# mayataka/robotoc

Hardware: AMD Instinct MI355X
Metric: riccati_sweeps_per_sec (higher is better)
Workload: dtype f64; 1 GPU; anymal_trot_N40 (nv=18,nu=12, 47 grids: 2 lifts + 2 impacts, switching constraints ns=6), 4096 DISTINCT OCP instances per GPU (randomised stage data and dx0), backward+forward Riccati sweep; per_gpu_batch=4096, stages=47, parallelism=instances sharded, dp1

## Files before the change

robotoc_amd/csrc/kernel_set.hpp:

```cpp
#pragma once
#include <cstring>

#include "../../include/rtoc.h"
#include "condense.hpp"
#include "state_equation.hpp"
#include "unconstr_dynamics.hpp"
#include "friction_cone.hpp"
#include "kkt_error.hpp"
#include "integrate_solution.hpp"
#include "riccati_backward.hpp"
#include "riccati_backward_rs.hpp"
#include "riccati_backward_rv.hpp"
#include "riccati_backward_rw.hpp"
#include "riccati_backward_rw2.hpp"
#include "condense_rv.hpp"
#include "riccati_scan.hpp"
#include "riccati_forward.hpp"
#include "unconstr_riccati.hpp"

namespace rtoc {

typedef void (*bwd_fn)(BwdArgs);
typedef void (*fwd_fn)(FwdArgs);
typedef void (*fill_fn)(FillArgs);
typedef void (*ud_fn)(UdArgs);
typedef void (*cone_fn)(ConeArgs);
typedef void (*cond_fn)(CondArgs);
typedef void (*expd_fn)(ExpArgs);
typedef void (*scan_fn)(ScanArgs);
typedef void (*fscan_fn)(FwdScanArgs);
typedef void (*stoscan_fn)(StoScanArgs);
typedef void (*ur_fn)(UrArgs);
constexpr size_t kernel_abi_stamp() {
  size_t h = 1469598103934665603ull;
  const size_t parts[] = {sizeof(BwdArgs), sizeof(FwdArgs), sizeof(FillArgs), sizeof(UdArgs), sizeof(ConeArgs), sizeof(CondArgs),
                          sizeof(ExpArgs), sizeof(ScanArgs), sizeof(FwdScanArgs), sizeof(UrArgs), sizeof(StoScanArgs)};
  for (size_t v : parts) h = (h ^ v) * 1099511628211ull;
  return h;
}

struct KernelSet {
  int nv, nu, ns;
  int nvariants;
  bwd_fn bwd[4];
  int bwd_waves[4];
  int bwd_lds[4];
  int bwd_inst[4];
  bwd_fn bwd_sa;
  bwd_fn bwd_rv;
  bwd_fn bwd_rv_sa;
  bwd_fn bwd_rv_sto;
  int bwd_rv_lds;
  bwd_fn bwd_rw;
  int bwd_rw_lds;
  int bwd_rw_threads;
  rtoc_record_layout kl, rl, dl, cl;
  fwd_fn fwd;
  int fwd_threads;
  fill_fn fill;
  ud_fn ucond, uexp;
  ur_fn ubwd, ufwd;
  cone_fn ccond, cexp;
  cone_fn wcond, wexp;
  cond_fn cond;
  cond_fn cond_split, mjt;
  int mjt_lds;
  int cond_threads, cond_lds, cond_split_lds;
  int cond_fuses_cones;
  int cond_fused_default;
  cond_fn cond_rv_nc;
  cond_fn cond_rv;
  int cond_rv_lds;
  int cond_rv_cones;
  expd_fn expd;
  int expd_threads, expd_lds;
  scan_fn scan_elt, scan_comb;
  int scan_elt_lds, scan_comb_lds, scan_comb_threads;
  int scan_elt_stride, scan_ps_stride, scan_ps_soff;
  int scan_policy_variant;
  fscan_fn fscan_elt, fscan_comb, fscan_fin;
  int fscan_lds;
  stoscan_fn sto_prep, sto_vec;
  int sto_prep_lds, sto_vec_lds, sto_vec_threads, sto_scr_stride;
};

template <int NV, int NU, int NS, int NW0, int NW1>
inline KernelSet make_set() {
  KernelSet k;
  memset(&k, 0, sizeof(k));
  k.nv = NV;
  k.nu = NU;
  k.ns = NS;
  k.nvariants = 2;
  for (int v = 0; v < 4; ++v) k.bwd_inst[v] = 1;
  k.kl = StaticLayout<NV, NU, NS>::make().kkt;
  k.rl = StaticLayout<NV, NU, NS>::make().ric;
  k.bwd[0] = riccati_backward_kernel<NV, NU, NS, NW0>;
  k.bwd_waves[0] = NW0;
  k.bwd_lds[0] = BwdCfg<NV, NU, NS, NW0>::LDS_BYTES;
  k.bwd[1] = riccati_backward_kernel<NV, NU, NS, NW1>;
  k.bwd_waves[1] = NW1;
  k.bwd_lds[1] = BwdCfg<NV, NU, NS, NW1>::LDS_BYTES;
  if constexpr (2 * NV + 1 <= 64 && NU + 3 <= 16) {
    k.bwd[2] = riccati_backward_rs_kernel<NV, NU, NS>;
    k.bwd_waves[2] = 2;
    k.bwd_lds[2] = BwdCfg<NV, NU, NS, 2>::LDS_BYTES;
    k.nvariants = 3;
    if (4 * BwdCfg<NV, NU, NS, 2>::LDS_BYTES + 64 <= 160 * 1024) {
      k.bwd[3] = riccati_backward_rs4_kernel<NV, NU, NS>;
      k.bwd_waves[3] = 8;
      k.bwd_lds[3] = 4 * BwdCfg<NV, NU, NS, 2>::LDS_BYTES + 64;
      k.bwd_inst[3] = 4;
      k.nvariants = 4;
      if constexpr (NV % 4 == 2 && NV > NU) k.bwd_sa = riccati_backward_rs4_kernel<NV, NU, NS, true>;
    }
  }
  if constexpr (RvCfg<NV, NU>::OK) {
    k.bwd_rv = riccati_backward_rv_kernel<NV, NU, NS, false>;
    if constexpr (NV % 16 == 2 && RvCfg<NV, NU>::T == 3 && NV - NU > 0 && NV - NU <= 8 && (NV - NU) % 2 == 0)
    {
      k.bwd_rv_sa = riccati_backward_rv_kernel<NV, NU, NS, true>;
      k.bwd_rv_sto = riccati_backward_rv_kernel<NV, NU, NS, true, true>;
    }
    k.bwd_rv_lds = rv_lds_bytes<NV, NU, NS>();
  }
  if constexpr (RwCfg<NV, NU>::OK) {
    k.bwd_rw = riccati_backward_rw_kernel<NV, NU, NS>;
    k.bwd_rw_lds = RwLds<NV, NU, NS>::BYTES;
    k.bwd_rw_threads = 64;
  } else if constexpr (RwCfg<NV, NU>::OK2) {
    k.bwd_rw = riccati_backward_rw2_kernel<NV, NU, NS>;
    k.bwd_rw_lds = Rw2Lds<NV, NU, NS>::BYTES;
    k.bwd_rw_threads = 128;
  }
  constexpr int NWF = (2 * NV + NU + 63) / 64;
  if constexpr (NWF == 1)
    k.fwd = riccati_forward_kernel<NV, NU, NS, 1>;
  else
    k.fwd = riccati_forward_mw_kernel<NV, NU, NS, NWF>;
  k.fwd_threads = 64 * NWF;
  k.dl = StaticLayout<NV, NU, NS>::make().dir;
  k.cl = StaticLayout<NV, NU, NS>::make().cdd;
  k.fill = unconstr_fill_kernel<NV>;
  k.ucond = unconstr_condense_kernel<NV>;
  k.uexp = unconstr_expand_kernel<NV>;
  if constexpr (NU == NV && NS == 0 && 2 * NV + 1 <= 64) {
    if constexpr (NV <= 8) k.ubwd = unconstr_riccati_backward_kernel<NV>;
    else k.ubwd = unconstr_riccati_backward_lds_kernel<NV>;
    k.ufwd = unconstr_riccati_forward_kernel<NV>;
  }
  k.ccond = cone_condense_kernel<NV, NS>;
  k.cexp = cone_expand_kernel<NV, NS>;
  k.wcond = wrench_condense_kernel<NV, NS>;
  k.wexp = wrench_expand_kernel<NV, NS>;
  constexpr int NF = NS;
  k.cond = condense_kernel<NV, NU, NF, NS>;
  k.cond_split = condense_kernel<NV, NU, NF, NS, true>;
  k.mjt = mjtjinv_kernel<NV, NU, NF, NS>;
  k.mjt_lds = MjCfg<NV, NF>::LDS_BYTES;
  k.cond_threads = CondCfg<NV, NU, NF, NS>::NT;
  k.cond_lds = CondCfg<NV, NU, NF, NS>::LDS_BYTES;
  k.cond_split_lds = CondCfg<NV, NU, NF, NS, true>::LDS_BYTES;
  k.cond_fuses_cones = CondCfg<NV, NU, NF, NS>::FUSE ? 1 : 0;
  k.cond_fused_default = (CondCfg<NV, NU, NF, NS>::FUSE && CondCfg<NV, NU, NF, NS>::ITEMS >= 5) ? 1 : 0;
  k.cond_rv = nullptr;
  k.cond_rv_nc = nullptr;
  k.cond_rv_lds = 0;
  k.cond_rv_cones = 0;
  if constexpr (CrvCfg<NV, NU, NF, NS>::OK) {
    k.cond_rv = condense_rv_kernel<NV, NU, NF, NS>;
    k.cond_rv_nc = condense_rv_kernel<NV, NU, NF, NS, false>;
    k.cond_rv_lds = CrvCfg<NV, NU, NF, NS>::LDS_BYTES;
    k.cond_rv_cones = CrvCfg<NV, NU, NF, NS>::CONES ? 1 : 0;
  }
  static_assert(!(NV == 18 && NU == 12 && NS == 12) ||
                    (CondCfg<NV, NU, NF, NS, true>::ITEMS >= 5 && CondCfg<NV, NU, NF, NS, true>::MIN_WAVES == 4 && MjCfg<NV, NF>::ITEMS >= 10),
                "LDS carve of the split condensation grew past its granule budget");
  k.expd = expand_kernel<NV, NU, NF, NS>;
  k.expd_threads = 64;
  k.expd_lds = ExpCfg<NV, NU, NF>::LDS_BYTES;
  k.scan_elt = scan_element_kernel<NV, NU, NS>;
  k.scan_comb = scan_combine_kernel<NV>;
  k.scan_elt_lds = scan::ElementCfg<NV, NU, NS>::LDS_BYTES;
  k.scan_comb_threads = scan_comb_nt(NV);
  k.scan_comb_lds = scan::CombineCfg<NV, scan_comb_nt(NV)>::LDS_BYTES;
  k.scan_elt_stride = scan::EltLayout<NV>::STRIDE;
  k.scan_ps_stride = scan::EltLayout<NV>::PS_STRIDE;
  k.scan_ps_soff = scan::EltLayout<NV>::PS_S;
  k.scan_policy_variant = 1;
  k.fscan_elt = fwd_scan_element_kernel<NV, NU, NS>;
  k.fscan_comb = fwd_scan_combine_kernel<NV, NU, NS>;
  k.fscan_fin = fwd_scan_finish_kernel<NV, NU, NS>;
  k.fscan_lds = scan::FwdCfg<NV, NU>::LDS_BYTES;
  k.sto_prep = scan_sto_prep_kernel<NV, NU, NS>;
  k.sto_vec = scan_sto_vector_kernel<NV, NU, NS>;
  k.sto_prep_lds = scan::StoPrepCfg<NV, NU, NS>::LDS_DOUBLES * (int)sizeof(double);
  k.sto_vec_lds = scan::StoVecCfg<NV, NU, NS>::LDS_BYTES;
  k.sto_vec_threads = scan_sto_vec_nt(NV);
  k.sto_scr_stride = scan::StoScratch<NV, NU, NS>::STRIDE;
  static_assert(scan::StoVecCfg<NV, NU, NS>::LDS_BYTES <= 160 * 1024, "the vector pass keeps one grid point's bundle in LDS");
  static_assert(scan::CombineCfg<NV, scan_comb_nt(NV)>::LDS_BYTES <= 160 * 1024, "combination scratch must fit the LDS of a CU");
  return k;
}


}
```

robotoc_amd/csrc/riccati_forward.hpp:

```cpp
#pragma once
#include "device_utils.hpp"
#include "../../include/rtoc.h"

namespace rtoc {

#ifndef FWD_UNROLL
#define FWD_UNROLL 18
#endif
#ifndef FWD_REST_PARTS
#define FWD_REST_PARTS 2
#endif
#ifndef FWD_HEAD
#define FWD_HEAD 8
#endif

struct FwdArgs {
  const double* kkt;
  const double* ric;
  double* dir;
  const double* dx0;
  const rtoc_grid* grid;
  int nstages;
  int batch;
  int first;
};

template <int NWF>
__device__ __forceinline__ void fwd_sync() {
  if constexpr (NWF == 1)
    asm volatile("s_waitcnt lgkmcnt(0)" ::: "memory");
  else
    asm volatile("s_waitcnt lgkmcnt(0)\n\ts_barrier" ::: "memory");
}

template <int NV, int NU, int NS, int NWF>
__global__ __launch_bounds__(64 * NWF, 4) void riccati_forward_kernel(FwdArgs a) {
  constexpr int NX = 2 * NV, NT = 64 * NWF;
  constexpr bool MFOLD = NS > 0 && NX + NU + NS <= NT;
  static_assert(NX + NU <= NT, "one thread per row of [Fxx;K]");
  __shared__ double sDx[2][NX + 8];
  __shared__ double sDu[NU + 8];
  __shared__ double sRed[8];
  extern __shared__ int sGridTab[];
  const int tid = threadIdx.x;
  const int b = a.first + blockIdx.x;
  if (b >= a.batch) return;
  for (int st = tid; st < a.nstages; st += NT) {
    const rtoc_grid* gp = a.grid + st;
    sGridTab[st] = (gp->type & 15) | ((gp->sto != 0) << 4) | ((gp->sto_next != 0) << 5) |
                   ((gp->switching_constraint != 0) << 6) | (gp->dims << 8);
  }
  const int N = a.nstages - 1;
  constexpr rtoc_layout SL = StaticLayout<NV, NU, NS>::make();
  constexpr rtoc_record_layout KL = SL.kkt, RL = SL.ric, DL = SL.dir;
  const double* kb = a.kkt + (size_t)b * a.nstages * KL.stride;
  const double* rb = a.ric + (size_t)b * a.nstages * RL.stride;
  double* db = a.dir + (size_t)b * a.nstages * DL.stride;

  if (tid < NX) {
    const double v = a.dx0 ? a.dx0[(size_t)b * NX + tid] : db[DL.off[RTOC_DIR_DX] + tid];
    sDx[0][tid] = v;
    if (a.dx0) db[DL.off[RTOC_DIR_DX] + tid] = v;
  }
  __syncthreads();
  double dts = 0.0, dtsn = 0.0;
  {
    const rtoc_grid g0 = a.grid[0];
    if (g0.sto) {
      if (tid == 0) {
        double acc = 0.0;
        for (int k = 0; k < NX; ++k) acc += rb[RL.off[RTOC_RIC_DTSDX] + k] * sDx[0][k];
        sRed[0] = acc + rb[RL.off[RTOC_RIC_SCAL] + RTOC_RIC_SCAL_DTS0];
      }
      __syncthreads();
      dtsn = sRed[0];
      __syncthreads();
    }
  }
  int cur = 0;
  struct GridBits { int type, sto, sto_next, switching_constraint, dims; };
  struct StageRows {
    const double *pa, *pp, *pv, *ps;
    int sa;
  };
  auto stage_rows = [&](int st) {
    const int gb = __builtin_amdgcn_readfirstlane(sGridTab[st]);
    const bool imp = (gb & 15) == RTOC_GRID_IMPACT;
    const bool xrow = tid < NX;
    const bool krow = !imp && tid >= NX && tid < NX + NU;
    const bool mrow = MFOLD && ((gb >> 6) & 1) && tid >= NX + NU && tid < NX + NU + (gb >> 8);
    const int u = krow ? tid - NX : 0;
    const int m = mrow ? tid - NX - NU : 0;
    const int t = xrow ? tid : 0;
    const double* kr = kb + (size_t)st * KL.stride;
    const double* rr = rb + (size_t)st * RL.stride;
    StageRows r;
    r.pa = xrow ? kr + KL.off[RTOC_KKT_FXX] + tid
                : (mrow ? rr + RL.off[RTOC_RIC_M] + m : rr + RL.off[RTOC_RIC_K] + (size_t)u * NX);
    r.sa = xrow ? NX : (mrow ? NS : 1);
    r.pp = rr + RL.off[RTOC_RIC_P] + t;
    r.pv = xrow ? kr + KL.off[RTOC_KKT_FX] + tid : (mrow ? rr + RL.off[RTOC_RIC_MV] + m : rr + RL.off[RTOC_RIC_KV] + u);
    r.ps = rr + RL.off[RTOC_RIC_S] + t;
    return r;
  };
  constexpr int H = NX < FWD_HEAD ? NX : FWD_HEAD;
  double ha[H], hp[H], vec, sv;
  {
    const StageRows r0 = stage_rows(0);
#pragma unroll
    for (int j = 0; j < H; ++j) {
      ha[j] = r0.pa[j * r0.sa];
      hp[j] = r0.pp[j * NX];
    }
    vec = *r0.pv;
    sv = *r0.ps;
  }
  for (int st = 0; st < N; ++st) {
    const int gb = __builtin_amdgcn_readfirstlane(sGridTab[st]);
    const GridBits g = {gb & 15, (gb >> 4) & 1, (gb >> 5) & 1, (gb >> 6) & 1, gb >> 8};
    const bool impact = g.type == RTOC_GRID_IMPACT, lift = g.type == RTOC_GRID_LIFT;
    const bool sto = g.sto != 0, sto_next = g.sto_next != 0;
    const double* kr = kb + (size_t)st * KL.stride;
    const double* rr = rb + (size_t)st * RL.stride;
    double* dr = db + (size_t)st * DL.stride;
    const double* dx = sDx[cur];
    double* dxn = sDx[cur ^ 1];

    if (impact || lift) {
      dts = dtsn;
      dtsn = 0.0;
      if (lift && sto_next) {
        if (tid == 0) {
          double acc = 0.0;
          for (int k = 0; k < NX; ++k) acc += rr[RL.off[RTOC_RIC_DTSDX] + k] * dx[k];
          acc += rr[RL.off[RTOC_RIC_SCAL] + RTOC_RIC_SCAL_DTS0];
          if (sto) acc += rr[RL.off[RTOC_RIC_SCAL] + RTOC_RIC_SCAL_DTSDTS] * dts;
          sRed[0] = acc;
        }
        fwd_sync<NWF>();
        dtsn = sRed[0];
        fwd_sync<NWF>();
      }
    }

    const bool xrow = tid < NX;
    const bool krow = !impact && tid >= NX && tid < NX + NU;
    const bool mrow = MFOLD && g.switching_constraint && tid >= NX + NU && tid < NX + NU + g.dims;
    const int u = krow ? tid - NX : 0;
    const int m = mrow ? tid - NX - NU : 0;
    const StageRows r = stage_rows(st);
    double bv[NU];
    double acc_a = 0.0, acc_p = 0.0;
#pragma unroll
    for (int j = 0; j < H; ++j) {
      const double x = dx[j];
      acc_a += ha[j] * x;
      acc_p += hp[j] * x;
    }
#pragma unroll((NX - H + FWD_REST_PARTS - 1) / FWD_REST_PARTS > 0 ? (NX - H + FWD_REST_PARTS - 1) / FWD_REST_PARTS : 1)
    for (int j = H; j < NX; ++j) {
      const double x = dx[j];
      acc_a += r.pa[j * r.sa] * x;
      acc_p += r.pp[j * NX] * x;
    }
    {
      const double* Bv = kr + KL.off[RTOC_KKT_FVU] + ((tid >= NV && tid < NX) ? tid - NV : 0);
#pragma unroll
      for (int c = 0; c < NU; ++c) bv[c] = Bv[c * NV];
    }
    double vec_n, sv_n;
    {
      const StageRows rn = stage_rows(st + 1);
#pragma unroll
      for (int j = 0; j < H; ++j) {
        ha[j] = rn.pa[j * rn.sa];
        hp[j] = rn.pp[j * NX];
      }
      vec_n = *rn.pv;
      sv_n = *rn.ps;
    }
    if (krow) {
      double du = acc_a + vec;
      if (sto) {
        du += rr[RL.off[RTOC_RIC_T] + u] * (dtsn - dts);
        if (sto_next) du -= rr[RL.off[RTOC_RIC_W] + u] * dtsn;
      }
      sDu[u] = du;
      dr[DL.off[RTOC_DIR_DU] + u] = du;
    }
    fwd_sync<NWF>();
    if (xrow) {
      double v = vec + acc_a;
      if (!impact) {
        if (tid >= NV) {
#pragma unroll
          for (int c = 0; c < NU; ++c) v += bv[c] * sDu[c];
        }
        if (sto) v += kr[KL.off[RTOC_KKT_FFX] + tid] * (dtsn - dts);
      }
      dxn[tid] = v;
      (dr + DL.stride)[DL.off[RTOC_DIR_DX] + tid] = v;
    }
    if (impact && sto_next) {
      fwd_sync<NWF>();
      if (tid == 0) {
        double acc = 0.0;
        for (int k = 0; k < NX; ++k) acc += rr[RL.off[RTOC_RIC_DTSDX] + k] * dxn[k];
        acc += rr[RL.off[RTOC_RIC_SCAL] + RTOC_RIC_SCAL_DTS0];
        if (sto) acc += rr[RL.off[RTOC_RIC_SCAL] + RTOC_RIC_SCAL_DTSDTS] * dts;
        sRed[0] = acc;
      }
      fwd_sync<NWF>();
      dtsn = sRed[0];
    }
    if (tid < NX) {
      double lam = acc_p - sv;
      if (sto) {
        if (impact) {
          lam -= rr[RL.off[RTOC_RIC_PHI] + tid] * dtsn;
        } else {
          lam += rr[RL.off[RTOC_RIC_PSI] + tid] * (dtsn - dts);
          if (sto_next) lam -= rr[RL.off[RTOC_RIC_PHI] + tid] * dtsn;
        }
      }
      dr[DL.off[RTOC_DIR_DLMDGMM] + tid] = lam;
    }
    if constexpr (MFOLD) {
      if (mrow) {
        double acc = acc_a + vec;
        if (sto) {
          acc += rr[RL.off[RTOC_RIC_MT] + m] * (dtsn - dts);
          if (sto_next) acc -= rr[RL.off[RTOC_RIC_MTN] + m] * dtsn;
        }
        dr[DL.off[RTOC_DIR_DXI] + m] = acc;
      }
    } else if (NS > 0 && g.switching_constraint && tid < g.dims) {
      const double* M = rr + RL.off[RTOC_RIC_M] + tid;
      double acc = 0.0;
      for (int j = 0; j < NX; ++j) acc += M[j * NS] * dx[j];
      acc += rr[RL.off[RTOC_RIC_MV] + tid];
      if (sto) {
        acc += rr[RL.off[RTOC_RIC_MT] + tid] * (dtsn - dts);
        if (sto_next) acc -= rr[RL.off[RTOC_RIC_MTN] + tid] * dtsn;
      }
      dr[DL.off[RTOC_DIR_DXI] + tid] = acc;
    }
    if (tid == 0) {
      dr[DL.off[RTOC_DIR_DTS] + 0] = dts;
      dr[DL.off[RTOC_DIR_DTS] + 1] = dtsn;
    }
    fwd_sync<NWF>();
    cur ^= 1;
    vec = vec_n;
    sv = sv_n;
  }
  {
    const double* rr = rb + (size_t)N * RL.stride;
    double* dr = db + (size_t)N * DL.stride;
    const double* dx = sDx[cur];
    if (tid < NX) {
      const double* P = rr + RL.off[RTOC_RIC_P] + tid;
      double acc = 0.0;
#pragma unroll FWD_UNROLL
      for (int j = 0; j < NX; ++j) acc += P[j * NX] * dx[j];
      dr[DL.off[RTOC_DIR_DLMDGMM] + tid] = acc - rr[RL.off[RTOC_RIC_S] + tid];
    }
    if (tid == 0) {
      dr[DL.off[RTOC_DIR_DTS] + 0] = dts;
      dr[DL.off[RTOC_DIR_DTS] + 1] = dtsn;
    }
  }
}

template <int NV, int NU, int NS, int NWF>
__global__ __launch_bounds__(64 * NWF) void riccati_forward_mw_kernel(FwdArgs a) {
  constexpr int NX = 2 * NV, NT = 64 * NWF;
  static_assert(NX + NU <= NT, "one thread per row of [Fxx;K]");
  __shared__ double sDx[2][NX + 8];
  __shared__ double sDu[NU + 8];
  __shared__ double sRed[8];
  const int tid = threadIdx.x;
  const int b = a.first + blockIdx.x;
  if (b >= a.batch) return;
  const int N = a.nstages - 1;
  constexpr rtoc_layout SL = StaticLayout<NV, NU, NS>::make();
  constexpr rtoc_record_layout KL = SL.kkt, RL = SL.ric, DL = SL.dir;
  const double* kb = a.kkt + (size_t)b * a.nstages * KL.stride;
  const double* rb = a.ric + (size_t)b * a.nstages * RL.stride;
  double* db = a.dir + (size_t)b * a.nstages * DL.stride;

  if (tid < NX) {
    const double v = a.dx0 ? a.dx0[(size_t)b * NX + tid] : db[DL.off[RTOC_DIR_DX] + tid];
    sDx[0][tid] = v;
    if (a.dx0) db[DL.off[RTOC_DIR_DX] + tid] = v;
  }
  __syncthreads();
  double dts = 0.0, dtsn = 0.0;
  {
    const rtoc_grid g0 = a.grid[0];
    if (g0.sto) {
      if (tid == 0) {
        double acc = 0.0;
        for (int k = 0; k < NX; ++k) acc += rb[RL.off[RTOC_RIC_DTSDX] + k] * sDx[0][k];
        sRed[0] = acc + rb[RL.off[RTOC_RIC_SCAL] + RTOC_RIC_SCAL_DTS0];
      }
      __syncthreads();
      dtsn = sRed[0];
      __syncthreads();
    }
  }
  int cur = 0;
  for (int st = 0; st < N; ++st) {
    const rtoc_grid g = a.grid[st];
    const bool impact = g.type == RTOC_GRID_IMPACT, lift = g.type == RTOC_GRID_LIFT;
    const bool sto = g.sto != 0, sto_next = g.sto_next != 0;
    const double* kr = kb + (size_t)st * KL.stride;
    const double* rr = rb + (size_t)st * RL.stride;
    double* dr = db + (size_t)st * DL.stride;
    const double* dx = sDx[cur];
    double* dxn = sDx[cur ^ 1];

    if (impact || lift) {
      dts = dtsn;
      dtsn = 0.0;
      if (lift && sto_next) {
        if (tid == 0) {
          double acc = 0.0;
          for (int k = 0; k < NX; ++k) acc += rr[RL.off[RTOC_RIC_DTSDX] + k] * dx[k];
          acc += rr[RL.off[RTOC_RIC_SCAL] + RTOC_RIC_SCAL_DTS0];
          if (sto) acc += rr[RL.off[RTOC_RIC_SCAL] + RTOC_RIC_SCAL_DTSDTS] * dts;
          sRed[0] = acc;
        }
        __syncthreads();
        dtsn = sRed[0];
        __syncthreads();
      }
    }

    double acc_a = 0.0, acc_p = 0.0;
    if (tid < NX) {
      const double* A = kr + KL.off[RTOC_KKT_FXX] + tid;
      const double* P = rr + RL.off[RTOC_RIC_P] + tid;
#pragma unroll FWD_UNROLL
      for (int j = 0; j < NX; ++j) {
        const double x = dx[j];
        acc_a += A[j * NX] * x;
        acc_p += P[j * NX] * x;
      }
    } else if (!impact && tid < NX + NU) {
      const int u = tid - NX;
      const double* K = rr + RL.off[RTOC_RIC_K] + (size_t)u * NX;
#pragma unroll 6
      for (int j = 0; j < NX; ++j) acc_a += K[j] * dx[j];
      double du = acc_a + rr[RL.off[RTOC_RIC_KV] + u];
      if (sto) {
        du += rr[RL.off[RTOC_RIC_T] + u] * (dtsn - dts);
        if (sto_next) du -= rr[RL.off[RTOC_RIC_W] + u] * dtsn;
      }
      sDu[u] = du;
      dr[DL.off[RTOC_DIR_DU] + u] = du;
    }
    __syncthreads();
    if (tid < NX) {
      double v = kr[KL.off[RTOC_KKT_FX] + tid] + acc_a;
      if (!impact) {
        if (tid >= NV) {
          const double* Bv = kr + KL.off[RTOC_KKT_FVU] + (tid - NV);
#pragma unroll 4
          for (int u = 0; u < NU; ++u) v += Bv[u * NV] * sDu[u];
        }
        if (sto) v += kr[KL.off[RTOC_KKT_FFX] + tid] * (dtsn - dts);
      }
      dxn[tid] = v;
      (dr + DL.stride)[DL.off[RTOC_DIR_DX] + tid] = v;
    }
    if (impact && sto_next) {
      __syncthreads();
      if (tid == 0) {
        double acc = 0.0;
        for (int k = 0; k < NX; ++k) acc += rr[RL.off[RTOC_RIC_DTSDX] + k] * dxn[k];
        acc += rr[RL.off[RTOC_RIC_SCAL] + RTOC_RIC_SCAL_DTS0];
        if (sto) acc += rr[RL.off[RTOC_RIC_SCAL] + RTOC_RIC_SCAL_DTSDTS] * dts;
        sRed[0] = acc;
      }
      __syncthreads();
      dtsn = sRed[0];
    }
    if (tid < NX) {
      double lam = acc_p - rr[RL.off[RTOC_RIC_S] + tid];
      if (sto) {
        if (impact) {
          lam -= rr[RL.off[RTOC_RIC_PHI] + tid] * dtsn;
        } else {
          lam += rr[RL.off[RTOC_RIC_PSI] + tid] * (dtsn - dts);
          if (sto_next) lam -= rr[RL.off[RTOC_RIC_PHI] + tid] * dtsn;
        }
      }
      dr[DL.off[RTOC_DIR_DLMDGMM] + tid] = lam;
    }
    if (NS > 0 && g.switching_constraint && tid < g.dims) {
      const double* M = rr + RL.off[RTOC_RIC_M] + tid;
      double acc = 0.0;
      for (int j = 0; j < NX; ++j) acc += M[j * NS] * dx[j];
      acc += rr[RL.off[RTOC_RIC_MV] + tid];
      if (sto) {
        acc += rr[RL.off[RTOC_RIC_MT] + tid] * (dtsn - dts);
        if (sto_next) acc -= rr[RL.off[RTOC_RIC_MTN] + tid] * dtsn;
      }
      dr[DL.off[RTOC_DIR_DXI] + tid] = acc;
    }
    if (tid == 0) {
      dr[DL.off[RTOC_DIR_DTS] + 0] = dts;
      dr[DL.off[RTOC_DIR_DTS] + 1] = dtsn;
    }
    __syncthreads();
    cur ^= 1;
  }
  {
    const double* rr = rb + (size_t)N * RL.stride;
    double* dr = db + (size_t)N * DL.stride;
    const double* dx = sDx[cur];
    if (tid < NX) {
      const double* P = rr + RL.off[RTOC_RIC_P] + tid;
      double acc = 0.0;
#pragma unroll 6
      for (int j = 0; j < NX; ++j) acc += P[j * NX] * dx[j];
      dr[DL.off[RTOC_DIR_DLMDGMM] + tid] = acc - rr[RL.off[RTOC_RIC_S] + tid];
    }
    if (tid == 0) {
      dr[DL.off[RTOC_DIR_DTS] + 0] = dts;
      dr[DL.off[RTOC_DIR_DTS] + 1] = dtsn;
    }
  }
}

struct FillArgs {
  double* kkt;
  int nstages, batch;
  double dt;
  rtoc_record_layout kl;
};

template <int NV>
__global__ void unconstr_fill_kernel(FillArgs a) {
  constexpr int NX = 2 * NV;
  const int rec = blockIdx.x;
  if (rec >= a.batch * a.nstages) return;
  double* r = a.kkt + (size_t)rec * a.kl.stride;
  double* A = r + a.kl.off[RTOC_KKT_FXX];
  double* Bv = r + a.kl.off[RTOC_KKT_FVU];
  for (int e = threadIdx.x; e < NX * NX; e += blockDim.x) {
    const int i = e % NX, j = e / NX;
    double v = (i == j) ? 1.0 : 0.0;
    if (i < NV && j == i + NV) v = a.dt;
    A[e] = v;
  }
  for (int e = threadIdx.x; e < NV * NV; e += blockDim.x) {
    const int i = e % NV, j = e / NV;
    Bv[e] = (i == j) ? a.dt : 0.0;
  }
}

}
```

Baseline: 1.359 million sweeps/s.

## Split forward Riccati mat-vecs across all lanes with paired loads and LDS reduction

```diff
diff --git a/robotoc_amd/csrc/kernel_set.hpp b/robotoc_amd/csrc/kernel_set.hpp
--- a/robotoc_amd/csrc/kernel_set.hpp
+++ b/robotoc_amd/csrc/kernel_set.hpp
@@ -135,7 +135,7 @@
   }
   constexpr int NWF = (2 * NV + NU + 63) / 64;
   if constexpr (NWF == 1)
-    k.fwd = riccati_forward_kernel<NV, NU, NS, 1>;
+    k.fwd = riccati_forward_kernel<NV, NU, NS>;
   else
     k.fwd = riccati_forward_mw_kernel<NV, NU, NS, NWF>;
   k.fwd_threads = 64 * NWF;
diff --git a/robotoc_amd/csrc/riccati_forward.hpp b/robotoc_amd/csrc/riccati_forward.hpp
--- a/robotoc_amd/csrc/riccati_forward.hpp
+++ b/robotoc_amd/csrc/riccati_forward.hpp
@@ -3,16 +3,6 @@
 #include "../../include/rtoc.h"
 
 namespace rtoc {
-
-#ifndef FWD_UNROLL
-#define FWD_UNROLL 18
-#endif
-#ifndef FWD_REST_PARTS
-#define FWD_REST_PARTS 2
-#endif
-#ifndef FWD_HEAD
-#define FWD_HEAD 8
-#endif
 
 struct FwdArgs {
   const double* kkt;
@@ -25,6 +15,25 @@
   int first;
 };
 
+#ifndef FWD_PREFETCH
+#define FWD_PREFETCH 12
+#endif
+#ifndef FWD_WAVES_PER_SIMD
+#define FWD_WAVES_PER_SIMD 2
+#endif
+
+template <int NV, int NU>
+struct FwdPairCfg {
+  static constexpr int NX = 2 * NV;
+  static constexpr int G = 64 / NV;
+  static constexpr int TX = (NX + G - 1) / G;
+  static constexpr int TXP = (TX + 1) & ~1;
+  static constexpr int TK = (NU + G - 1) / G;
+  static constexpr int NVP = (NV + 1) & ~1;
+  static constexpr int NF = NV * NU, NFP = (NF + 1) & ~1;
+  static constexpr int TF = (NFP + 127) / 128;
+};
+
 template <int NWF>
 __device__ __forceinline__ void fwd_sync() {
   if constexpr (NWF == 1)
@@ -33,23 +42,31 @@
     asm volatile("s_waitcnt lgkmcnt(0)\n\ts_barrier" ::: "memory");
 }
 
-template <int NV, int NU, int NS, int NWF>
-__global__ __launch_bounds__(64 * NWF, 4) void riccati_forward_kernel(FwdArgs a) {
-  constexpr int NX = 2 * NV, NT = 64 * NWF;
-  constexpr bool MFOLD = NS > 0 && NX + NU + NS <= NT;
-  static_assert(NX + NU <= NT, "one thread per row of [Fxx;K]");
-  __shared__ double sDx[2][NX + 8];
+template <int NV, int NU, int NS>
+__global__ __launch_bounds__(64, FWD_WAVES_PER_SIMD) void riccati_forward_kernel(FwdArgs a) {
+  using C = FwdPairCfg<NV, NU>;
+  constexpr int NX = C::NX, G = C::G, TX = C::TX, TXP = C::TXP, TK = C::TK, NVP = C::NVP, NF = C::NF, TF = C::TF;
+  constexpr int PF = FWD_PREFETCH < TX ? FWD_PREFETCH : TX;
+  static_assert(NX + NU <= 64, "one lane per row of [Fxx; K] in the reductions");
+  __shared__ __attribute__((aligned(16))) double sDx[2][NX + 8];
+  __shared__ __attribute__((aligned(16))) double sXp[2][G * TXP];
+  __shared__ __attribute__((aligned(16))) double sPa[G + 1][NX];
+  __shared__ __attribute__((aligned(16))) double sPp[G + 1][NX];
+  __shared__ __attribute__((aligned(16))) double sPk[NU + 1][NVP];
+  __shared__ __attribute__((aligned(16))) double sF[TF * 128];
   __shared__ double sDu[NU + 8];
+  __shared__ double sDt[NX];
   __shared__ double sRed[8];
   extern __shared__ int sGridTab[];
   const int tid = threadIdx.x;
   const int b = a.first + blockIdx.x;
   if (b >= a.batch) return;
-  for (int st = tid; st < a.nstages; st += NT) {
+  for (int st = tid; st < a.nstages; st += 64) {
     const rtoc_grid* gp = a.grid + st;
     sGridTab[st] = (gp->type & 15) | ((gp->sto != 0) << 4) | ((gp->sto_next != 0) << 5) |
                    ((gp->switching_constraint != 0) << 6) | (gp->dims << 8);
   }
+  for (int e = tid; e < 2 * G * TXP; e += 64) (&sXp[0][0])[e] = 0.0;
   const int N = a.nstages - 1;
   constexpr rtoc_layout SL = StaticLayout<NV, NU, NS>::make();
   constexpr rtoc_record_layout KL = SL.kkt, RL = SL.ric, DL = SL.dir;
@@ -57,9 +74,20 @@
   const double* rb = a.ric + (size_t)b * a.nstages * RL.stride;
   double* db = a.dir + (size_t)b * a.nstages * DL.stride;
 
-  if (tid < NX) {
+  const bool lg = tid < G * NV;
+  const int p = lg ? tid % NV : tid - G * NV;
+  const int c = lg ? tid / NV : 0;
+  const int cw = lg ? c : G;
+  const bool xrow = tid < NX;
+  const int r = xrow ? tid : NX - 1;
+  const bool kl = tid >= NX && tid < NX + NU;
+  const int u = kl ? tid - NX : 0;
+  const int pos = (r % G) * TXP + r / G;
+  __syncthreads();
+  if (xrow) {
     const double v = a.dx0 ? a.dx0[(size_t)b * NX + tid] : db[DL.off[RTOC_DIR_DX] + tid];
     sDx[0][tid] = v;
+    sXp[0][pos] = v;
     if (a.dx0) db[DL.off[RTOC_DIR_DX] + tid] = v;
   }
   __syncthreads();
@@ -77,44 +105,23 @@
       __syncthreads();
     }
   }
+  const int lo = c * NX + 2 * p;
+  auto moff = [&](int t) { return (NX % G == 0 || t < TX - 1 || G * t + c < NX) ? lo + t * (G * NX) : (NX - 1) * NX + 2 * p; };
+  auto live = [&](int t) { return NX % G == 0 || t < TX - 1 || G * t + c < NX; };
+  auto koff = [&](int t) { return (NU % G == 0 || t < TK - 1 || G * t + c < NU) ? lo + t * (G * NX) : (NU - 1) * NX + 2 * p; };
+  auto klive = [&](int t) { return NU % G == 0 || t < TK - 1 || G * t + c < NU; };
+  auto vec_ptr = [&](int st) {
+    return xrow ? kb + (size_t)st * KL.stride + KL.off[RTOC_KKT_FX] + tid : rb + (size_t)st * RL.stride + RL.off[RTOC_RIC_KV] + u;
+  };
+  auto s_ptr = [&](int st) { return rb + (size_t)st * RL.stride + RL.off[RTOC_RIC_S] + r; };
+  d2 fa[TX];
+  double vec, sv;
+#pragma unroll
+  for (int t = 0; t < PF; ++t) fa[t] = *(const d2*)(kb + KL.off[RTOC_KKT_FXX] + moff(t));
+  vec = *vec_ptr(0);
+  sv = *s_ptr(0);
   int cur = 0;
   struct GridBits { int type, sto, sto_next, switching_constraint, dims; };
-  struct StageRows {
-    const double *pa, *pp, *pv, *ps;
-    int sa;
-  };
-  auto stage_rows = [&](int st) {
-    const int gb = __builtin_amdgcn_readfirstlane(sGridTab[st]);
-    const bool imp = (gb & 15) == RTOC_GRID_IMPACT;
-    const bool xrow = tid < NX;
-    const bool krow = !imp && tid >= NX && tid < NX + NU;
-    const bool mrow = MFOLD && ((gb >> 6) & 1) && tid >= NX + NU && tid < NX + NU + (gb >> 8);
-    const int u = krow ? tid - NX : 0;
-    const int m = mrow ? tid - NX - NU : 0;
-    const int t = xrow ? tid : 0;
-    const double* kr = kb + (size_t)st * KL.stride;
-    const double* rr = rb + (size_t)st * RL.stride;
-    StageRows r;
-    r.pa = xrow ? kr + KL.off[RTOC_KKT_FXX] + tid
-                : (mrow ? rr + RL.off[RTOC_RIC_M] + m : rr + RL.off[RTOC_RIC_K] + (size_t)u * NX);
-    r.sa = xrow ? NX : (mrow ? NS : 1);
-    r.pp = rr + RL.off[RTOC_RIC_P] + t;
-    r.pv = xrow ? kr + KL.off[RTOC_KKT_FX] + tid : (mrow ? rr + RL.off[RTOC_RIC_MV] + m : rr + RL.off[RTOC_RIC_KV] + u);
-    r.ps = rr + RL.off[RTOC_RIC_S] + t;
-    return r;
-  };
-  constexpr int H = NX < FWD_HEAD ? NX : FWD_HEAD;
-  double ha[H], hp[H], vec, sv;
-  {
-    const StageRows r0 = stage_rows(0);
-#pragma unroll
-    for (int j = 0; j < H; ++j) {
-      ha[j] = r0.pa[j * r0.sa];
-      hp[j] = r0.pp[j * NX];
-    }
-    vec = *r0.pv;
-    sv = *r0.ps;
-  }
   for (int st = 0; st < N; ++st) {
     const int gb = __builtin_amdgcn_readfirstlane(sGridTab[st]);
     const GridBits g = {gb & 15, (gb >> 4) & 1, (gb >> 5) & 1, (gb >> 6) & 1, gb >> 8};
@@ -124,7 +131,7 @@
     const double* rr = rb + (size_t)st * RL.stride;
     double* dr = db + (size_t)st * DL.stride;
     const double* dx = sDx[cur];
-    double* dxn = sDx[cur ^ 1];
+    const double* xp = sXp[cur];
 
     if (impact || lift) {
       dts = dtsn;
@@ -132,111 +139,153 @@
       if (lift && sto_next) {
         if (tid == 0) {
           double acc = 0.0;
+          #pragma unroll 4
           for (int k = 0; k < NX; ++k) acc += rr[RL.off[RTOC_RIC_DTSDX] + k] * dx[k];
           acc += rr[RL.off[RTOC_RIC_SCAL] + RTOC_RIC_SCAL_DTS0];
           if (sto) acc += rr[RL.off[RTOC_RIC_SCAL] + RTOC_RIC_SCAL_DTSDTS] * dts;
           sRed[0] = acc;
         }
-        fwd_sync<NWF>();
+        fwd_sync<1>();
         dtsn = sRed[0];
-        fwd_sync<NWF>();
-      }
-    }
-
-    const bool xrow = tid < NX;
-    const bool krow = !impact && tid >= NX && tid < NX + NU;
-    const bool mrow = MFOLD && g.switching_constraint && tid >= NX + NU && tid < NX + NU + g.dims;
-    const int u = krow ? tid - NX : 0;
-    const int m = mrow ? tid - NX - NU : 0;
-    const StageRows r = stage_rows(st);
-    double bv[NU];
-    double acc_a = 0.0, acc_p = 0.0;
-#pragma unroll
-    for (int j = 0; j < H; ++j) {
-      const double x = dx[j];
-      acc_a += ha[j] * x;
-      acc_p += hp[j] * x;
-    }
-#pragma unroll((NX - H + FWD_REST_PARTS - 1) / FWD_REST_PARTS > 0 ? (NX - H + FWD_REST_PARTS - 1) / FWD_REST_PARTS : 1)
-    for (int j = H; j < NX; ++j) {
-      const double x = dx[j];
-      acc_a += r.pa[j * r.sa] * x;
-      acc_p += r.pp[j * NX] * x;
-    }
+        fwd_sync<1>();
+      }
+    }
+
+    d2 fk[TK], ff[TF], fp[TX];
+#pragma unroll
+    for (int t = PF; t < TX; ++t) fa[t] = *(const d2*)(kr + KL.off[RTOC_KKT_FXX] + moff(t));
+#pragma unroll
+    for (int t = 0; t < TK; ++t) fk[t] = *(const d2*)(rr + RL.off[RTOC_RIC_K] + koff(t));
+#pragma unroll
+    for (int i = 0; i < TF; ++i) {
+      const int e = 2 * (64 * i + tid);
+      ff[i] = *(const d2*)(kr + KL.off[RTOC_KKT_FVU] + (e < NF ? e : 0));
+    }
+    double rd1 = 0.0, rd2 = 0.0, rd3 = 0.0, rdt = 0.0, rs0 = 0.0, rss = 0.0;
+    if (sto) {
+      rd1 = xrow ? kr[KL.off[RTOC_KKT_FFX] + tid] : rr[RL.off[RTOC_RIC_T] + u];
+      rd2 = xrow ? rr[RL.off[RTOC_RIC_PSI] + tid] : rr[RL.off[RTOC_RIC_W] + u];
+      rd3 = rr[RL.off[RTOC_RIC_PHI] + r];
+    }
+    if (impact && sto_next) {
+      rdt = rr[RL.off[RTOC_RIC_DTSDX] + r];
+      rs0 = rr[RL.off[RTOC_RIC_SCAL] + RTOC_RIC_SCAL_DTS0];
+      rss = rr[RL.off[RTOC_RIC_SCAL] + RTOC_RIC_SCAL_DTSDTS];
+    }
+    d2 x[TXP / 2];
+#pragma unroll
+    for (int i = 0; i < TXP / 2; ++i) x[i] = *(const d2*)(xp + c * TXP + 2 * i);
+    const d2 xq = *(const d2*)(dx + 2 * p);
+    double a0 = 0.0, a1 = 0.0;
+#pragma unroll
+    for (int t = 0; t < TX; ++t) {
+      const double xt = x[t / 2][t % 2];
+      if (live(t)) {
+        a0 += fa[t].x * xt;
+        a1 += fa[t].y * xt;
+      }
+    }
+    __builtin_amdgcn_sched_barrier(0);
+#pragma unroll
+    for (int t = 0; t < TX; ++t) fp[t] = *(const d2*)(rr + RL.off[RTOC_RIC_P] + moff(t));
+    double pk[TK];
+#pragma unroll
+    for (int t = 0; t < TK; ++t) pk[t] = fk[t].x * xq.x + fk[t].y * xq.y;
+#pragma unroll
+    for (int i = 0; i < TF; ++i) *(d2*)(sF + 2 * (64 * i + tid)) = ff[i];
+    double q0 = 0.0, q1 = 0.0;
+#pragma unroll
+    for (int t = 0; t < TX; ++t) {
+      const double xt = x[t / 2][t % 2];
+      if (live(t)) {
+        q0 += fp[t].x * xt;
+        q1 += fp[t].y * xt;
+      }
+    }
+    double vec_n, sv_n;
+    __builtin_amdgcn_sched_barrier(0);
     {
-      const double* Bv = kr + KL.off[RTOC_KKT_FVU] + ((tid >= NV && tid < NX) ? tid - NV : 0);
-#pragma unroll
-      for (int c = 0; c < NU; ++c) bv[c] = Bv[c * NV];
-    }
-    double vec_n, sv_n;
+      const double* kn = kb + (size_t)(st + 1) * KL.stride;
+#pragma unroll
+      for (int t = 0; t < PF; ++t) fa[t] = *(const d2*)(kn + KL.off[RTOC_KKT_FXX] + moff(t));
+      vec_n = *vec_ptr(st + 1);
+      sv_n = *s_ptr(st + 1);
+    }
     {
-      const StageRows rn = stage_rows(st + 1);
-#pragma unroll
-      for (int j = 0; j < H; ++j) {
-        ha[j] = rn.pa[j * rn.sa];
-        hp[j] = rn.pp[j * NX];
-      }
-      vec_n = *rn.pv;
-      sv_n = *rn.ps;
-    }
-    if (krow) {
-      double du = acc_a + vec;
+      d2 va = {a0, a1}, vp = {q0, q1};
+      *(d2*)(&sPa[cw][2 * p]) = va;
+      *(d2*)(&sPp[cw][2 * p]) = vp;
+#pragma unroll
+      for (int t = 0; t < TK; ++t) sPk[lg && klive(t) ? G * t + c : NU][p] = pk[t];
+    }
+    fwd_sync<1>();
+    double acc_a = sPa[0][r], acc_p = sPp[0][r];
+#pragma unroll
+    for (int cc = 1; cc < G; ++cc) {
+      acc_a += sPa[cc][r];
+      acc_p += sPp[cc][r];
+    }
+    double kd = 0.0;
+#pragma unroll 3
+    for (int i = 0; i < NVP / 2; ++i) {
+      const d2 w = *(const d2*)(&sPk[u][2 * i]);
+      kd += w.x;
+      if (2 * i + 1 < NV) kd += w.y;
+    }
+    if (kl && !impact) {
+      double du = kd + vec;
       if (sto) {
-        du += rr[RL.off[RTOC_RIC_T] + u] * (dtsn - dts);
-        if (sto_next) du -= rr[RL.off[RTOC_RIC_W] + u] * dtsn;
+        du += rd1 * (dtsn - dts);
+        if (sto_next) du -= rd2 * dtsn;
       }
       sDu[u] = du;
       dr[DL.off[RTOC_DIR_DU] + u] = du;
     }
-    fwd_sync<NWF>();
+    fwd_sync<1>();
+    double* dxn = sDx[cur ^ 1];
     if (xrow) {
       double v = vec + acc_a;
       if (!impact) {
         if (tid >= NV) {
-#pragma unroll
-          for (int c = 0; c < NU; ++c) v += bv[c] * sDu[c];
+#pragma unroll 4
+          for (int cc = 0; cc < NU; ++cc) v += sF[cc * NV + tid - NV] * sDu[cc];
         }
-        if (sto) v += kr[KL.off[RTOC_KKT_FFX] + tid] * (dtsn - dts);
+        if (sto) v += rd1 * (dtsn - dts);
       }
       dxn[tid] = v;
+      if (impact && sto_next) sDt[tid] = rdt;
+      sXp[cur ^ 1][pos] = v;
       (dr + DL.stride)[DL.off[RTOC_DIR_DX] + tid] = v;
     }
     if (impact && sto_next) {
-      fwd_sync<NWF>();
+      fwd_sync<1>();
       if (tid == 0) {
         double acc = 0.0;
-        for (int k = 0; k < NX; ++k) acc += rr[RL.off[RTOC_RIC_DTSDX] + k] * dxn[k];
-        acc += rr[RL.off[RTOC_RIC_SCAL] + RTOC_RIC_SCAL_DTS0];
-        if (sto) acc += rr[RL.off[RTOC_RIC_SCAL] + RTOC_RIC_SCAL_DTSDTS] * dts;
+        #pragma unroll 4
+        for (int k = 0; k < NX; ++k) acc += sDt[k] * dxn[k];
+        acc += rs0;
+        if (sto) acc += rss * dts;
         sRed[0] = acc;
       }
-      fwd_sync<NWF>();
+      fwd_sync<1>();
       dtsn = sRed[0];
     }
-    if (tid < NX) {
+    if (xrow) {
       double lam = acc_p - sv;
       if (sto) {
         if (impact) {
-          lam -= rr[RL.off[RTOC_RIC_PHI] + tid] * dtsn;
+          lam -= rd3 * dtsn;
         } else {
-          lam += rr[RL.off[RTOC_RIC_PSI] + tid] * (dtsn - dts);
-          if (sto_next) lam -= rr[RL.off[RTOC_RIC_PHI] + tid] * dtsn;
+          lam += rd2 * (dtsn - dts);
+          if (sto_next) lam -= rd3 * dtsn;
         }
       }
       dr[DL.off[RTOC_DIR_DLMDGMM] + tid] = lam;
     }
-    if constexpr (MFOLD) {
-      if (mrow) {
-        double acc = acc_a + vec;
-        if (sto) {
-          acc += rr[RL.off[RTOC_RIC_MT] + m] * (dtsn - dts);
-          if (sto_next) acc -= rr[RL.off[RTOC_RIC_MTN] + m] * dtsn;
-        }
-        dr[DL.off[RTOC_DIR_DXI] + m] = acc;
-      }
-    } else if (NS > 0 && g.switching_constraint && tid < g.dims) {
+    if (NS > 0 && g.switching_constraint && tid < g.dims) {
       const double* M = rr + RL.off[RTOC_RIC_M] + tid;
       double acc = 0.0;
+      #pragma unroll 4
       for (int j = 0; j < NX; ++j) acc += M[j * NS] * dx[j];
       acc += rr[RL.off[RTOC_RIC_MV] + tid];
       if (sto) {
@@ -249,7 +298,7 @@
       dr[DL.off[RTOC_DIR_DTS] + 0] = dts;
       dr[DL.off[RTOC_DIR_DTS] + 1] = dtsn;
     }
-    fwd_sync<NWF>();
+    fwd_sync<1>();
     cur ^= 1;
     vec = vec_n;
     sv = sv_n;
@@ -257,14 +306,30 @@
   {
     const double* rr = rb + (size_t)N * RL.stride;
     double* dr = db + (size_t)N * DL.stride;
-    const double* dx = sDx[cur];
-    if (tid < NX) {
-      const double* P = rr + RL.off[RTOC_RIC_P] + tid;
-      double acc = 0.0;
-#pragma unroll FWD_UNROLL
-      for (int j = 0; j < NX; ++j) acc += P[j * NX] * dx[j];
-      dr[DL.off[RTOC_DIR_DLMDGMM] + tid] = acc - rr[RL.off[RTOC_RIC_S] + tid];
-    }
+    const double* xp = sXp[cur];
+    d2 fp[TX], x[TXP / 2];
+#pragma unroll
+    for (int t = 0; t < TX; ++t) fp[t] = *(const d2*)(rr + RL.off[RTOC_RIC_P] + moff(t));
+#pragma unroll
+    for (int i = 0; i < TXP / 2; ++i) x[i] = *(const d2*)(xp + c * TXP + 2 * i);
+    double q0 = 0.0, q1 = 0.0;
+#pragma unroll
+    for (int t = 0; t < TX; ++t) {
+      const double xt = x[t / 2][t % 2];
+      if (live(t)) {
+        q0 += fp[t].x * xt;
+        q1 += fp[t].y * xt;
+      }
+    }
+    {
+      d2 vp = {q0, q1};
+      *(d2*)(&sPp[cw][2 * p]) = vp;
+    }
+    fwd_sync<1>();
+    double acc_p = sPp[0][r];
+#pragma unroll
+    for (int cc = 1; cc < G; ++cc) acc_p += sPp[cc][r];
+    if (xrow) dr[DL.off[RTOC_DIR_DLMDGMM] + tid] = acc_p - sv;
     if (tid == 0) {
       dr[DL.off[RTOC_DIR_DTS] + 0] = dts;
       dr[DL.off[RTOC_DIR_DTS] + 1] = dtsn;
@@ -341,7 +406,7 @@
     if (tid < NX) {
       const double* A = kr + KL.off[RTOC_KKT_FXX] + tid;
       const double* P = rr + RL.off[RTOC_RIC_P] + tid;
-#pragma unroll FWD_UNROLL
+#pragma unroll 18
       for (int j = 0; j < NX; ++j) {
         const double x = dx[j];
         acc_a += A[j * NX] * x;
```

Result: faster. 1.413 million sweeps/s, median of 6 (+4.0%).
